# Amos-Chen98/neo-planner

Measured on NVIDIA B200. Metric: optimized trajectories/sec to convergence, higher is better.
Workload: dtype f64

## Files before the change

### neo_planner_b200/csrc/lbfgsb_tile.cuh

```cuda
#pragma once
#include "minco_tile.cuh"
#include "x87_nrm2.h"

namespace neo {

#ifdef NEO_OPT_TICKS
#define OT_BEGIN long long ot_last = clock64()
#define OT(i) do { const long long ot_now = clock64(); if (T.tl == 0) { atomicAdd((unsigned long long *)&g_opt_ticks[i], (unsigned long long)(ot_now - ot_last)); atomicAdd((unsigned long long *)&g_opt_ticks[32 + (i)], 1ull); } ot_last = clock64(); } while (0)
#else
#define OT_BEGIN do { } while (0)
#define OT(i) do { } while (0)
#endif

__device__ __forceinline__ double xmul(double a, double b) { return __dmul_rn(a, b); }
__device__ __forceinline__ double xadd(double a, double b) { return __dadd_rn(a, b); }
__device__ __forceinline__ double xsub(double a, double b) { return __dsub_rn(a, b); }
__device__ __noinline__ double xdiv(double a, double b) { return __ddiv_rn(a, b); }
__device__ __noinline__ double xsqrt(double a) { return __dsqrt_rn(a); }
__device__ __noinline__ double nrm2_x87(int n, const double *v) { return x87_nrm2(n, v); }
__device__ __forceinline__ double xrcp(double a) { return __drcp_rn(a); }
__device__ __forceinline__ double xfma(double a, double b, double c) { return __fma_rn(a, b, c); }
__device__ __forceinline__ double xdiv_r(double a, double b, double rb)
{
    const double q = __dmul_rn(a, rb);
    return __fma_rn(__fma_rn(-b, q, a), rb, q);
}

struct Dcsrch {
    bool brackt;
    int stage;
    double finit, ginit, gtest, width, width1, stx, fx, gx, sty, fy, gy, stmin, stmax;
};

#define LS_FTOL 1e-3
#define LS_GTOL 0.9
#define LS_XTOL 0.1
#define LS_STPMIN 0.0
#define LS_STPMAX 1e10

__device__ __forceinline__ double max3(double a, double b, double c) { return fmax(a, fmax(b, c)); }

__device__ __forceinline__ void dcstep(double &stx, double &fx, double &dx, double &sty, double &fy, double &dy, double &stp,
                                       double fp, double dp, bool &brackt, double stpmin, double stpmax)
{
    const double sgnd = xmul(dp, dx > 0.0 ? 1.0 : (dx < 0.0 ? -1.0 : __longlong_as_double(0x7ff8000000000000LL)));
    const int kase = fp > fx ? 1 : (sgnd < 0.0 ? 2 : (fabs(dp) < fabs(dx) ? 3 : 4));
    const bool cubic = kase < 4 || brackt;
    const double fa = kase < 4 ? fx : fp, fb = kase < 4 ? fp : fy, da = kase < 4 ? dx : dy;
    const double den = kase < 4 ? xsub(stp, stx) : xsub(sty, stp);
    double theta = 0.0, gamma = 0.0, rden = 0.0;
    if (cubic) {
        rden = __drcp_rn(den);
        theta = xadd(xadd(xdiv_r(xmul(3.0, xsub(fa, fb)), den, rden), da), dp);
        const double s = max3(fabs(theta), fabs(da), fabs(dp));
        const double rs = __drcp_rn(s);
        const double ts = xdiv_r(theta, s, rs);
        double rad = xsub(xmul(ts, ts), xmul(xdiv_r(da, s, rs), xdiv_r(dp, s, rs)));
        if (kase == 3) rad = fmax(0.0, rad);
        gamma = xmul(s, __dsqrt_rn(rad));
        const bool flip = kase == 1 ? stp < stx : (kase == 4 ? stp > sty : stp > stx);
        if (flip) gamma = -gamma;
    }
    const double g1 = xsub(gamma, kase == 1 ? dx : dp);
    const double p = xadd(g1, theta);
    const double q = kase == 3 ? xadd(xadd(gamma, xsub(dx, dp)), gamma) : xadd(xadd(g1, gamma), kase == 1 ? dp : (kase == 2 ? dx : dy));
    const double r = cubic ? __ddiv_rn(p, q) : 0.0;
    const double qn = kase == 1 ? dx : dp;
    const double qd = kase == 1 ? xadd(xdiv_r(xsub(fx, fp), den, rden), dx) : xsub(dp, dx);
    const double qq = kase < 4 ? __ddiv_rn(qn, qd) : 0.0;
    double stpf, stpc, stpq;
    if (kase == 1) {
        stpc = xadd(stx, xmul(r, den));
        stpq = xadd(stx, xmul(xmul(qq, 0.5), den));
        if (fabs(xsub(stpc, stx)) < fabs(xsub(stpq, stx))) stpf = stpc; else stpf = xadd(stpc, xmul(xsub(stpq, stpc), 0.5));
        brackt = true;
    } else if (kase == 2) {
        stpc = xadd(stp, xmul(r, xsub(stx, stp)));
        stpq = xadd(stp, xmul(qq, xsub(stx, stp)));
        if (fabs(xsub(stpc, stp)) > fabs(xsub(stpq, stp))) stpf = stpc; else stpf = stpq;
        brackt = true;
    } else if (kase == 3) {
        if (r < 0.0 && gamma != 0.0) stpc = xadd(stp, xmul(r, xsub(stx, stp)));
        else if (stp > stx) stpc = stpmax;
        else stpc = stpmin;
        stpq = xadd(stp, xmul(qq, xsub(stx, stp)));
        if (brackt) {
            if (fabs(xsub(stpc, stp)) < fabs(xsub(stpq, stp))) stpf = stpc; else stpf = stpq;
            if (stp > stx) stpf = fmin(xadd(stp, xmul(0.66, xsub(sty, stp))), stpf);
            else stpf = fmax(xadd(stp, xmul(0.66, xsub(sty, stp))), stpf);
        } else {
            if (fabs(xsub(stpc, stp)) > fabs(xsub(stpq, stp))) stpf = stpc; else stpf = stpq;
            stpf = fmin(stpmax, stpf); stpf = fmax(stpmin, stpf);
        }
    } else {
        if (brackt) stpf = xadd(stp, xmul(r, xsub(sty, stp)));
        else if (stp > stx) stpf = stpmax;
        else stpf = stpmin;
    }
    if (fp > fx) { sty = stp; fy = fp; dy = dp; }
    else {
        if (sgnd < 0.0) { sty = stx; fy = fx; dy = dx; }
        stx = stp; fx = fp; dx = dp;
    }
    stp = stpf;
}

__device__ __forceinline__ void dcsrch_start(Dcsrch &S, double stp, double f, double g)
{
    S.brackt = false; S.stage = 1; S.finit = f; S.ginit = g; S.gtest = xmul(LS_FTOL, g);
    S.width = LS_STPMAX - LS_STPMIN; S.width1 = xmul(S.width, 2.0);
    S.stx = 0.0; S.fx = f; S.gx = g; S.sty = 0.0; S.fy = f; S.gy = g;
    S.stmin = 0.0; S.stmax = xadd(stp, xmul(4.0, stp));
}

__device__ __forceinline__ int dcsrch_step(Dcsrch &S, double &stp, double f, double g)
{
    const double ftest = xadd(S.finit, xmul(stp, S.gtest));
    int task = 0;
    if (S.stage == 1 && f <= ftest && g >= 0.0) S.stage = 2;
    if (S.brackt && (stp <= S.stmin || stp >= S.stmax)) task = 2;
    if (S.brackt && xsub(S.stmax, S.stmin) <= xmul(LS_XTOL, S.stmax)) task = 2;
    if (stp == LS_STPMAX && f <= ftest && g <= S.gtest) task = 2;
    if (stp == LS_STPMIN && (f > ftest || g >= S.gtest)) task = 2;
    if (f <= ftest && fabs(g) <= xmul(LS_GTOL, -S.ginit)) task = 1;
    if (task) return task;
    {
        const bool mod = S.stage == 1 && f <= S.fx && f > ftest;
        const double gt = mod ? S.gtest : 0.0;
        const double fm = xsub(f, xmul(stp, gt)), gm = xsub(g, gt);
        double fxm = xsub(S.fx, xmul(S.stx, gt)), fym = xsub(S.fy, xmul(S.sty, gt)), gxm = xsub(S.gx, gt), gym = xsub(S.gy, gt);
        dcstep(S.stx, fxm, gxm, S.sty, fym, gym, stp, fm, gm, S.brackt, S.stmin, S.stmax);
        S.fx = xadd(fxm, xmul(S.stx, gt)); S.fy = xadd(fym, xmul(S.sty, gt));
        S.gx = xadd(gxm, gt); S.gy = xadd(gym, gt);
    }
    if (S.brackt) {
        if (fabs(xsub(S.sty, S.stx)) >= xmul(0.66, S.width1)) stp = xadd(S.stx, xmul(0.5, xsub(S.sty, S.stx)));
        S.width1 = S.width; S.width = fabs(xsub(S.sty, S.stx));
    }
    if (S.brackt) { S.stmin = fmin(S.stx, S.sty); S.stmax = fmax(S.stx, S.sty); }
    else { S.stmin = xadd(stp, xmul(1.1, xsub(stp, S.stx))); S.stmax = xadd(stp, xmul(4.0, xsub(stp, S.stx))); }
    stp = fmax(stp, LS_STPMIN); stp = fmin(stp, LS_STPMAX);
    if ((S.brackt && (stp <= S.stmin || stp >= S.stmax)) || (S.brackt && xsub(S.stmax, S.stmin) <= xmul(LS_XTOL, S.stmax)))
        stp = S.stx;
    return 0;
}

__device__ __noinline__ double blas_ddot(int n, const double *a, const double *b)
{
    double s = 0.0;
    int i = 0;
    if (n >= 16) {
        double v[4];
#pragma unroll
        for (int l = 0; l < 4; l++)
            v[l] = xadd(xadd(xadd(xmul(a[l], b[l]), xmul(a[4 + l], b[4 + l])), xmul(a[8 + l], b[8 + l])), xmul(a[12 + l], b[12 + l]));
        s = xadd(xadd(v[0], v[2]), xadd(v[1], v[3]));
        i = 16;
    }
#pragma unroll 1
    for (; i < n; i++) s = xfma(a[i], b[i], s);
    return s;
}
__device__ __noinline__ double loop_dot(int n, const double *a, const double *b)
{
    double s = 0.0;
#pragma unroll 1
    for (int i = 0; i < n; i++) s = xadd(s, xmul(a[i], b[i]));
    return s;
}

template <int N>
__device__ __forceinline__ double loop_dot_n(const double *a, const double *b, int n = N)
{
    if constexpr (N > 0 && N <= 10) {
        double s = 0.0;
#pragma unroll
        for (int i = 0; i < N; i++) s = xadd(s, xmul(a[i], b[i]));
        return s;
    } else return loop_dot(n, a, b);
}
template <int N>
__device__ __forceinline__ double blas_ddot_n(const double *a, const double *b, int n = N)
{
    if constexpr (N > 0 && N <= 10) {
        double s = 0.0;
#pragma unroll
        for (int i = 0; i < N; i++) s = xfma(a[i], b[i], s);
        return s;
    } else return blas_ddot(n, a, b);
}

__device__ __forceinline__ int wn_col(int j) { return j * (j + 1) / 2; }

__device__ __noinline__ bool lb_potf2(int tl, int TL, unsigned mask, double *wn, double *rd, int o, int n)
{
#pragma unroll 1
    for (int j = 0; j < n; j++) {
        double *cj = wn + wn_col(o + j) + o;
        double dot = 0.0;
#pragma unroll 1
        for (int k = 0; k < j; k++) dot = xfma(cj[k], cj[k], dot);
        const int m1 = j & ~3, k3 = j - m1;
        double v[2];
#pragma unroll
        for (int q = 0; q < 2; q++) {
            const int i = j + 1 + tl + q * TL;
            v[q] = 0.0;
            if (i < n) {
                const double *ci = wn + wn_col(o + i) + o;
                double t = ci[j];
                if (m1) {
                    double a0 = xmul(ci[0], cj[0]), a1 = xmul(ci[1], cj[1]), a2 = xmul(ci[2], cj[2]), a3 = xmul(ci[3], cj[3]);
                    if (m1 == 8) {
                        a0 = xadd(a0, xmul(ci[4], cj[4])); a1 = xadd(a1, xmul(ci[5], cj[5]));
                        a2 = xadd(a2, xmul(ci[6], cj[6])); a3 = xadd(a3, xmul(ci[7], cj[7]));
                    }
                    t = xsub(t, xadd(xadd(a0, a2), xadd(a1, a3)));
                }
                if (k3 == 1) t = xfma(ci[m1], -cj[m1], t);
                else if (k3 == 2) t = xadd(t, xfma(ci[m1], -cj[m1], xmul(ci[m1 + 1], -cj[m1 + 1])));
                else if (k3 == 3) t = xadd(t, xfma(ci[m1 + 2], -cj[m1 + 2], xfma(ci[m1], -cj[m1], xmul(ci[m1 + 1], -cj[m1 + 1]))));
                v[q] = t;
            }
        }
        double ajj = xsub(cj[j], dot);
        if (!(ajj > 0.0)) return false;
        ajj = __dsqrt_rn(ajj);
        const double r = __drcp_rn(ajj);
        __syncwarp(mask);
        if (tl == 0) { cj[j] = ajj; rd[o + j] = r; }
#pragma unroll
        for (int q = 0; q < 2; q++) {
            const int i = j + 1 + tl + q * TL;
            if (i < n) wn[wn_col(o + i) + o + j] = xmul(v[q], r);
        }
        __syncwarp(mask);
    }
    return true;
}

struct LbMem {
    int col, head, iupdat;
    double theta;
};

__device__ __forceinline__ int lb_slot(const LbMem &L, int k) { const int s = L.head + k; return s >= HIST ? s - HIST : s; }

template <int TL, int NC>
__device__ __forceinline__ void lb_update(const Tile<TL> &T, const TileMem &m, int n, LbMem &L, double s, double y, double rr, double dr)
{
    OT_BEGIN;
    L.iupdat++;
    if (L.iupdat <= HIST) L.col = L.iupdat;
    else L.head = L.head + 1 == HIST ? 0 : L.head + 1;
    const int col = L.col, slot = lb_slot(L, col - 1);
    if (T.tl < n) { m.ws[slot * n + T.tl] = s; m.wy[slot * n + T.tl] = y; }
    L.theta = xdiv(rr, dr);
    if (T.tl == 0) m.dr[slot] = dr;
    T.sync();
    const double *ynew = m.wy + slot * n;
#pragma unroll 1
    for (int e = T.tl; e < 2 * col; e += TL) {
        if (e < col) {
            const int sj = lb_slot(L, e);
            m.yr[slot * HIST + sj] = loop_dot_n<NC>(ynew, m.wy + sj * n, n);
        } else {
            const int si = lb_slot(L, e - col);
            const double v = loop_dot_n<NC>(m.ws + si * n, ynew, n);
            if (si == slot) m.rzd[slot] = v; else m.yr[si * HIST + slot] = v;
        }
    }
    T.sync();
    OT(2);
}

template <int TL>
__device__ __forceinline__ bool lb_factor(const Tile<TL> &T, const TileMem &m, const LbMem &L)
{
    const int col = L.col;
    OT_BEGIN;
    const double theta = L.theta, rtheta = xrcp(theta);
    double *wn = m.wn, *rd = m.wn + wn_col(LBW) + LBW;
#pragma unroll 1
    for (int iy = T.tl; iy < col; iy += TL) {
        const int si = lb_slot(L, iy), is = col + iy;
        double *c1 = wn + wn_col(iy), *c2 = wn + wn_col(is);
#pragma unroll 1
        for (int jy = 0; jy <= iy; jy++) {
            const int sj = lb_slot(L, jy);
            double v = xdiv_r(m.yr[si * HIST + sj], theta, rtheta);
            if (jy == iy) v = xadd(v, m.dr[si]);
            c1[jy] = v;
            c2[col + jy] = 0.0;
        }
#pragma unroll 1
        for (int jy = 0; jy < iy; jy++) c2[jy] = -0.0;
#pragma unroll 1
        for (int jy = iy; jy < col; jy++) {
            const int sj = lb_slot(L, jy);
            c2[jy] = jy == iy ? m.rzd[si] : m.yr[si * HIST + sj];
        }
    }
    T.sync();
    OT(3);
    if (!lb_potf2(T.tl, TL, T.mask, wn, rd, 0, col)) return false;
    OT(4);
    if (col == 1) {
        if (T.tl == 0) wn[wn_col(1)] = xdiv_r(wn[wn_col(1)], wn[0], rd[0]);
    } else {
#pragma unroll 1
        for (int c = col + T.tl; c < 2 * col; c += TL) {
            double *b = wn + wn_col(c);
            int kk = 0;
#pragma unroll 1
            for (int bs = 8; bs > 0; bs >>= 1) {
                if (!(col & bs)) continue;
                if (kk > 0)
#pragma unroll 1
                    for (int i = kk; i < kk + bs; i++) {
                        const double *ui = wn + wn_col(i);
                        double acc = 0.0;
#pragma unroll 1
                        for (int k = 0; k < kk; k++) acc = xfma(ui[k], b[k], acc);
                        b[i] = xsub(b[i], acc);
                    }
#pragma unroll 1
                for (int i = kk; i < kk + bs; i++) {
                    b[i] = xmul(b[i], rd[i]);
#pragma unroll 1
                    for (int k = i + 1; k < kk + bs; k++) b[k] = xfma(-b[i], wn[wn_col(k) + i], b[k]);
                }
                kk += bs;
            }
        }
    }
    T.sync();
    OT(5);
#pragma unroll 1
    for (int e = T.tl; e < col * (col + 1) / 2; e += TL) {
        int jj = 0;
        while ((jj + 1) * (jj + 2) / 2 <= e) jj++;
        const int ii = e - jj * (jj + 1) / 2, js = col + jj, is = col + ii;
        wn[wn_col(js) + is] = xadd(wn[wn_col(js) + is], blas_ddot(col, wn + wn_col(is), wn + wn_col(js)));
    }
    T.sync();
    OT(6);
    const bool pd = lb_potf2(T.tl, TL, T.mask, wn, rd, col, col);
    OT(7);
    return pd;
}

template <int TL, int NC>
__device__ __forceinline__ double lb_step(const Tile<TL> &T, const TileMem &m, int n, const LbMem &L, double g)
{
    const int col = L.col, m2 = 2 * col;
    OT_BEGIN;
    const double theta = L.theta, rtheta = xrcp(theta);
    double *wn = m.wn, *wv = m.wn + wn_col(LBW), *rd = wv + LBW;
    double d = -g;
    if (T.tl < n) m.dv[T.tl] = d;
    T.sync();
#pragma unroll 1
    for (int e = T.tl; e < m2; e += TL)
        wv[e] = e < col ? loop_dot_n<NC>(m.wy + lb_slot(L, e) * n, m.dv, n) : xmul(theta, loop_dot_n<NC>(m.ws + lb_slot(L, e - col) * n, m.dv, n));
    T.sync();
    OT(8);
    {
        constexpr int RPL = (LBW + TL - 1) / TL;
        double s[RPL];
#pragma unroll
        for (int q = 0; q < RPL; q++) s[q] = 0.0;
#pragma unroll 1
        for (int k = 0; k < m2; k++) {
            if ((k & (TL - 1)) == T.tl) {
                double v = wv[k];
                if (k > 0) {
                    double sk = s[0];
#pragma unroll
                    for (int q = 1; q < RPL; q++) if (k / TL == q) sk = s[q];
                    v = xsub(v, sk);
                }
                wv[k] = xdiv_r(v, wn[wn_col(k) + k], rd[k]);
            }
            T.sync();
            const double bk = wv[k];
#pragma unroll
            for (int q = 0; q < RPL; q++) {
                const int r = T.tl + q * TL;
                if (r > k && r < m2) {
                    const double *ur = wn + wn_col(r);
                    if (r < 16 || k >= 16) s[q] = xfma(ur[k], bk, s[q]);
                    else if (k == 15) s[q] = blas_ddot(16, ur, wv);
                }
            }
        }
    }
    T.sync();
    OT(9);
#pragma unroll 1
    for (int i = T.tl; i < col; i += TL) wv[i] = -wv[i];
    T.sync();
#pragma unroll 1
    for (int i = m2 - 1; i >= 0; i--) {
        const double *ui = wn + wn_col(i);
        if (T.tl == 0) wv[i] = xdiv_r(wv[i], ui[i], rd[i]);
        T.sync();
        const double t = -wv[i];
#pragma unroll 1
        for (int k = T.tl; k < i; k += TL) wv[k] = xfma(t, ui[k], wv[k]);
        T.sync();
    }
    OT(10);
    if (T.tl < n) {
#pragma unroll 1
        for (int jy = 0; jy < col; jy++) {
            const int sj = lb_slot(L, jy);
            d = xadd(xadd(d, xdiv_r(xmul(m.wy[sj * n + T.tl], wv[jy]), theta, rtheta)), xmul(m.ws[sj * n + T.tl], wv[col + jy]));
        }
        d = xmul(d, rtheta);
    }
    T.sync();
    OT(11);
    return d;
}

template <int TL>
__device__ __forceinline__ void ls_load(const Tile<TL> &T, const double *p, Dcsrch &S)
{
    S.finit = p[0]; S.ginit = p[1]; S.gtest = p[2]; S.width = p[3]; S.width1 = p[4]; S.stx = p[5]; S.fx = p[6]; S.gx = p[7];
    S.sty = p[8]; S.fy = p[9]; S.gy = p[10]; S.stmin = p[11]; S.stmax = p[12];
    const int flags = (int)p[13];
    S.brackt = (flags & 1) != 0; S.stage = flags >> 1;
}
template <int TL>
__device__ __forceinline__ void ls_store(const Tile<TL> &T, double *p, const Dcsrch &S)
{
    T.sync();
    if (T.tl == 0) {
        p[0] = S.finit; p[1] = S.ginit; p[2] = S.gtest; p[3] = S.width; p[4] = S.width1; p[5] = S.stx; p[6] = S.fx; p[7] = S.gx;
        p[8] = S.sty; p[9] = S.fy; p[10] = S.gy; p[11] = S.stmin; p[12] = S.stmax;
        p[13] = (double)((S.brackt ? 1 : 0) | (S.stage << 1));
    }
    T.sync();
}

constexpr int ST_CANCELLED = 7;
constexpr int ST_RUNNING = -1;

struct OptState {
    double x, g, d, t, r, z, xlast;
    double f, stp, gd;
    LbMem L;
    int nit, nfev, ifun, status;
    bool first;
};

__device__ __forceinline__ void opt_begin(OptState &o, double x0l)
{
    o.x = x0l; o.g = 0.0; o.d = 0.0; o.t = 0.0; o.r = 0.0; o.z = 0.0; o.xlast = 0.0;
    o.f = 0.0; o.stp = 0.0; o.gd = 0.0;
    o.L.col = 0; o.L.head = 0; o.L.iupdat = 0; o.L.theta = 1.0;
    o.nit = 0; o.nfev = 0; o.ifun = 0; o.status = ST_RUNNING; o.first = true;
}

template <int TL>
__device__ __forceinline__ bool opt_same_point(const Tile<TL> &T, const OptState &o, int n)
{
    return !o.first && T.all(T.tl >= n || o.x == o.xlast);
}

template <int TL, int NC>
__device__ __forceinline__ double opt_gd(const Tile<TL> &T, const TileMem &m, int n, double g, double d)
{
    T.sync();
    if (T.tl < n) { m.gv[T.tl] = g; m.dv[T.tl] = d; }
    T.sync();
    return blas_ddot_n<NC>(m.gv, m.dv, n);
}

template <int TL, int NC>
__device__ __forceinline__ void opt_advance(const Tile<TL> &T, const TileMem &m, int n, OptState &o,
                                            const unsigned *cancel_word, unsigned cancel_mask)
{
    const bool mine = T.tl < n;
    const double pgtol = 1e-4, ftol = 1e-4, epsmch = 2.220446049250313e-16;
    const double tol = (ftol / epsmch) * epsmch;
    const int maxls = 20, maxiter = 15000, maxfun = 15000;
    bool new_dir;
    OT_BEGIN;
    if (o.first) {
        o.first = false;
        if (T.dmax(mine ? fabs(o.g) : 0.0) <= pgtol) { o.status = 1; return; }
        new_dir = true;
    } else {
        o.gd = opt_gd<TL, NC>(T, m, n, o.g, o.d);
        Dcsrch ls;
        ls_load(T, m.ls, ls);
        const int ls_task = dcsrch_step(ls, o.stp, o.f, o.gd);
        if (ls_task == 0) ls_store(T, m.ls, ls);
        OT(0);
        if (ls_task == 0) new_dir = false;
        else {
            o.nit++;
            if (cancel_mask) {
                unsigned w = 0;
                if (T.tl == 0) w = *reinterpret_cast<const volatile unsigned *>(cancel_word);
                if (T.shfl(w, 0) & cancel_mask) { o.status = ST_CANCELLED; return; }
            }
            if (T.dmax(mine ? fabs(o.g) : 0.0) <= pgtol) { o.status = 1; return; }
            const double fold = m.ls[14], gdold = m.ls[15];
            if (xsub(fold, o.f) <= xmul(tol, max3(fabs(fold), fabs(o.f), 1.0))) { o.status = 0; return; }
            if (o.nit >= maxiter || o.nfev > maxfun) { o.status = 3; return; }
            const double y = xsub(o.g, o.r);
            T.sync();
            if (mine) m.dv[T.tl] = y;
            T.sync();
            OT(12);
            const double nr = nrm2_x87(n, m.dv);
            const double rr = xmul(nr, nr);
            OT(1);
            double dr, ddum, s;
            if (o.stp == 1.0) { dr = xsub(o.gd, gdold); ddum = -gdold; s = o.d; }
            else { dr = xmul(xsub(o.gd, gdold), o.stp); s = xmul(o.d, o.stp); ddum = xmul(-gdold, o.stp); }
            if (!(dr <= xmul(epsmch, ddum))) lb_update<TL, NC>(T, m, n, o.L, s, y, rr, dr);
            new_dir = true;
        }
    }
    for (;;) {
        if (new_dir) {
            OT(15);
            if (o.L.col > 0 && !lb_factor(T, m, o.L)) { o.L.col = 0; o.L.head = 0; o.L.iupdat = 0; o.L.theta = 1.0; }
            if (o.L.col == 0) o.z = xsub(o.x, o.g);
            else o.z = xadd(o.x, lb_step<TL, NC>(T, m, n, o.L, o.g));
            o.d = mine ? xsub(o.z, o.x) : 0.0;
            T.sync();
            if (mine) m.dv[T.tl] = o.d;
            T.sync();
            OT(13);
            const double dnorm = nrm2_x87(n, m.dv);
            OT(1);
            o.stp = (o.nit == 0) ? fmin(xdiv(1.0, dnorm), LS_STPMAX) : 1.0;
            o.t = o.x; o.r = o.g;
            o.gd = opt_gd<TL, NC>(T, m, n, o.g, o.d);
            T.sync();
            if (T.tl == 0) { m.ls[14] = o.f; m.ls[15] = o.gd; }
            o.ifun = 0;
            if (o.gd >= 0.0) o.ifun = maxls + 1;
            else { Dcsrch ls; dcsrch_start(ls, o.stp, o.f, o.gd); ls_store(T, m.ls, ls); }
            OT(14);
        }
        o.ifun++;
        if (o.ifun - 1 < maxls) break;
        T.sync();
        o.x = o.t; o.g = o.r; o.f = m.ls[14];
        if (o.L.col == 0) { o.status = 2; return; }
        o.L.col = 0; o.L.head = 0; o.L.iupdat = 0; o.L.theta = 1.0;
        new_dir = true;
    }
    o.x = (o.stp == 1.0) ? o.z : xadd(xmul(o.stp, o.d), o.t);
}

}
```

Measured before the change: 2.450 million.

## Restructure Cholesky and triangular solves to cut warp barriers and pipeline direction update

Rewrites lb_potf2 so each lane keeps running squared-sum accumulators for the rows it owns, and the diagonal owner computes sqrt and reciprocal itself. This leaves one warp barrier per column instead of two and removes the serial per-column dot loop. The forward solve in lb_step now broadcasts each solved element with a shuffle instead of a shared-memory write plus sync. The final direction accumulation software-pipelines its loads one step ahead. Host-side harness files are added to check that results still match the oracle, since the new accumulation order must stay bitwise consistent.

Measured after the change: 2.413 million (median of 6 runs). 0.985x the previous value.

```diff
diff --git a/devtools/direction_host.cpp b/devtools/direction_host.cpp
--- /dev/null
+++ b/devtools/direction_host.cpp
@@ -0,0 +1,135 @@
+#include <cmath>
+#include <condition_variable>
+#include <cstdio>
+#include <cstdlib>
+#include <cstring>
+#include <mutex>
+#include <thread>
+#include <vector>
+
+#define __device__
+#define __host__
+#define __forceinline__ inline
+#define __noinline__ __attribute__((noinline))
+#define NEO_HOST_TILE
+
+static inline double __dmul_rn(double a, double b) { return a * b; }
+static inline double __dadd_rn(double a, double b) { return a + b; }
+static inline double __dsub_rn(double a, double b) { return a - b; }
+static inline double __ddiv_rn(double a, double b) { return a / b; }
+static inline double __drcp_rn(double a) { return 1.0 / a; }
+static inline double __dsqrt_rn(double a) { return std::sqrt(a); }
+static inline double __fma_rn(double a, double b, double c) { return std::fma(a, b, c); }
+static inline double __longlong_as_double(long long v) { double d; memcpy(&d, &v, sizeof d); return d; }
+
+namespace neo {
+constexpr int HIST = 10;
+constexpr int LBW = 2 * HIST;
+constexpr int WN_DOUBLES = LBW * (LBW + 1) / 2 + 2 * LBW + 2;
+
+struct LaneSeq {
+    std::mutex m;
+    std::condition_variable cv;
+    int TL = 0, turn = 0, arrived = 0, descending = 0;
+    long gen = 0;
+    double val[32] = {}, seen[32] = {};
+    int first() const { return descending ? TL - 1 : 0; }
+    int next(int lane) const { return descending ? lane - 1 : lane + 1; }
+    double exchange(int lane, double v, int src)
+    {
+        std::unique_lock<std::mutex> lk(m);
+        val[lane] = v;
+        const long g = gen;
+        if (++arrived == TL) {
+            arrived = 0; gen++;
+            for (int l = 0; l < TL; l++) seen[l] = val[l];
+            turn = first();
+        } else turn = next(lane);
+        cv.notify_all();
+        if (!cv.wait_for(lk, std::chrono::seconds(20), [&] { return gen != g && turn == lane; })) {
+            fprintf(stderr, "direction_host: lanes disagree on the number of tile barriers\n");
+            abort();
+        }
+        return seen[src];
+    }
+    void start(int lane)
+    {
+        std::unique_lock<std::mutex> lk(m);
+        cv.wait(lk, [&] { return turn == lane; });
+    }
+    void leave(int lane)
+    {
+        exchange(lane, 0.0, 0);
+        std::unique_lock<std::mutex> lk(m);
+        turn = next(lane);
+        cv.notify_all();
+    }
+};
+thread_local LaneSeq *t_seq = nullptr;
+thread_local int t_lane = 0;
+}
+
+#define __syncwarp(mask) ((void)(mask), (void)neo::t_seq->exchange(neo::t_lane, 0.0, 0))
+
+namespace neo {
+template <int TL>
+struct Tile {
+    int tl;
+    unsigned mask;
+    explicit Tile(int lane) : tl(lane), mask(~0u) {}
+    void sync() const { __syncwarp(mask); }
+    double shfl(double v, int src) const { return t_seq->exchange(tl, v, src); }
+};
+struct TileMem {
+    double *ws, *wy, *yr, *rzd, *dr, *gv, *dv, *ls, *wn;
+};
+}
+
+
+#include "../neo_planner_b200/csrc/lbfgsb_tile.cuh"
+
+template <int TL>
+static int run_tile(int descending, int n, int pairs, const double *s, const double *y, const double *rr, const double *dr,
+                    const double *g, double *wn_out, double *d)
+{
+    using namespace neo;
+    std::vector<double> ws(HIST * n), wy(HIST * n), yr(HIST * HIST), rzd(HIST), drv(HIST), gv(n), dv(n), ls(16), wn(WN_DOUBLES);
+    const TileMem m{ws.data(), wy.data(), yr.data(), rzd.data(), drv.data(), gv.data(), dv.data(), ls.data(), wn.data()};
+    LaneSeq seq;
+    seq.TL = TL; seq.descending = descending; seq.turn = seq.first();
+    int ok = 0;
+    std::vector<std::thread> lanes;
+    for (int lane = 0; lane < TL; lane++)
+        lanes.emplace_back([&, lane] {
+            t_seq = &seq; t_lane = lane;
+            seq.start(lane);
+            const Tile<TL> T(lane);
+            LbMem L{0, 0, 0, 1.0};
+            for (int k = 0; k < pairs; k++)
+                lb_update<TL, 0>(T, m, n, L, lane < n ? s[k * n + lane] : 0.0, lane < n ? y[k * n + lane] : 0.0, rr[k], dr[k]);
+            const bool pd = lb_factor(T, m, L);
+            if (pd) {
+                const double dl = lb_step<TL, 0>(T, m, n, L, lane < n ? g[lane] : 0.0);
+                if (lane < n) d[lane] = dl;
+            }
+            if (lane == 0) ok = pd;
+            if (lane == 0 && pd) {
+                for (int j = 0; j < 2 * L.col; j++)
+                    for (int i = 0; i <= j; i++) wn_out[i * LBW + j] = wn[wn_col(j) + i];
+            }
+            seq.leave(lane);
+        });
+    for (auto &t : lanes) t.join();
+    return ok;
+}
+
+extern "C" int device_direction(int TL, int descending, int n, int pairs, const double *s, const double *y,
+                                const double *rr, const double *dr, const double *g, double *wn, double *d)
+{
+    switch (TL) {
+        case 8: return run_tile<8>(descending, n, pairs, s, y, rr, dr, g, wn, d);
+        case 16: return run_tile<16>(descending, n, pairs, s, y, rr, dr, g, wn, d);
+        case 32: return run_tile<32>(descending, n, pairs, s, y, rr, dr, g, wn, d);
+    }
+    return -1;
+}
diff --git a/devtools/direction_oracle.c b/devtools/direction_oracle.c
--- /dev/null
+++ b/devtools/direction_oracle.c
@@ -0,0 +1,13 @@
+#include "../oracle/minco_oracle.c"
+
+int oracle_direction(int n, int pairs, const double *s, const double *y, const double *rr, const double *dr,
+                     const double *g, double *wn, double *d)
+{
+    static __thread lb_mem C;
+    lb_reset(&C, n);
+    for (int k = 0; k < pairs; k++) lb_update(&C, s + (size_t)k * n, y + (size_t)k * n, rr[k], dr[k]);
+    const int ok = lb_factor(&C);
+    memcpy(wn, C.wn, sizeof(C.wn));
+    if (ok) lb_step(&C, g, d);
+    return ok;
+}
diff --git a/neo_planner_b200/csrc/lbfgsb_tile.cuh b/neo_planner_b200/csrc/lbfgsb_tile.cuh
--- a/neo_planner_b200/csrc/lbfgsb_tile.cuh
+++ b/neo_planner_b200/csrc/lbfgsb_tile.cuh
@@ -1,5 +1,7 @@
 #pragma once
+#ifndef NEO_HOST_TILE
 #include "minco_tile.cuh"
+#endif
 #include "x87_nrm2.h"
 
 namespace neo {
@@ -194,20 +196,25 @@
 
 __device__ __noinline__ bool lb_potf2(int tl, int TL, unsigned mask, double *wn, double *rd, int o, int n)
 {
+    double dot0 = 0.0, dot1 = 0.0;
 #pragma unroll 1
     for (int j = 0; j < n; j++) {
-        double *cj = wn + wn_col(o + j) + o;
-        double dot = 0.0;
-#pragma unroll 1
-        for (int k = 0; k < j; k++) dot = xfma(cj[k], cj[k], dot);
+        if ((j & (TL - 1)) == tl) {
+            double *ujj = wn + wn_col(o + j) + o + j;
+            const double u = __dsqrt_rn(xsub(*ujj, j < TL ? dot0 : dot1));
+            *ujj = u;
+            rd[o + j] = __drcp_rn(u);
+        }
+        __syncwarp(mask);
+        const double *cj = wn + wn_col(o + j) + o;
+        if (!(cj[j] > 0.0)) return false;
+        const double r = rd[o + j];
         const int m1 = j & ~3, k3 = j - m1;
-        double v[2];
-#pragma unroll
+#pragma unroll 1
         for (int q = 0; q < 2; q++) {
-            const int i = j + 1 + tl + q * TL;
-            v[q] = 0.0;
-            if (i < n) {
-                const double *ci = wn + wn_col(o + i) + o;
+            const int i = tl + q * TL;
+            if (i > j && i < n) {
+                double *ci = wn + wn_col(o + i) + o;
                 double t = ci[j];
                 if (m1) {
                     double a0 = xmul(ci[0], cj[0]), a1 = xmul(ci[1], cj[1]), a2 = xmul(ci[2], cj[2]), a3 = xmul(ci[3], cj[3]);
@@ -220,21 +227,12 @@
                 if (k3 == 1) t = xfma(ci[m1], -cj[m1], t);
                 else if (k3 == 2) t = xadd(t, xfma(ci[m1], -cj[m1], xmul(ci[m1 + 1], -cj[m1 + 1])));
                 else if (k3 == 3) t = xadd(t, xfma(ci[m1 + 2], -cj[m1 + 2], xfma(ci[m1], -cj[m1], xmul(ci[m1 + 1], -cj[m1 + 1]))));
-                v[q] = t;
+                const double u = xmul(t, r);
+                ci[j] = u;
+                dot0 = xfma(u, u, dot0);
             }
-        }
-        double ajj = xsub(cj[j], dot);
-        if (!(ajj > 0.0)) return false;
-        ajj = __dsqrt_rn(ajj);
-        const double r = __drcp_rn(ajj);
-        __syncwarp(mask);
-        if (tl == 0) { cj[j] = ajj; rd[o + j] = r; }
-#pragma unroll
-        for (int q = 0; q < 2; q++) {
-            const int i = j + 1 + tl + q * TL;
-            if (i < n) wn[wn_col(o + i) + o + j] = xmul(v[q], r);
-        }
-        __syncwarp(mask);
+            const double t = dot0; dot0 = dot1; dot1 = t;
+        }
     }
     return true;
 }
@@ -277,6 +275,7 @@
 template <int TL>
 __device__ __forceinline__ bool lb_factor(const Tile<TL> &T, const TileMem &m, const LbMem &L)
 {
+    static_assert(2 * TL >= HIST, "lb_potf2 keeps at most two columns per lane");
     const int col = L.col;
     OT_BEGIN;
     const double theta = L.theta, rtheta = xrcp(theta);
@@ -372,6 +371,7 @@
         for (int q = 0; q < RPL; q++) s[q] = 0.0;
 #pragma unroll 1
         for (int k = 0; k < m2; k++) {
+            double bk = 0.0;
             if ((k & (TL - 1)) == T.tl) {
                 double v = wv[k];
                 if (k > 0) {
@@ -380,10 +380,11 @@
                     for (int q = 1; q < RPL; q++) if (k / TL == q) sk = s[q];
                     v = xsub(v, sk);
                 }
-                wv[k] = xdiv_r(v, wn[wn_col(k) + k], rd[k]);
+                bk = xdiv_r(v, wn[wn_col(k) + k], rd[k]);
+                wv[k] = bk;
             }
-            T.sync();
-            const double bk = wv[k];
+            bk = T.shfl(bk, k & (TL - 1));
+            if (k == 15 && m2 > 16) T.sync();
 #pragma unroll
             for (int q = 0; q < RPL; q++) {
                 const int r = T.tl + q * TL;
@@ -395,8 +396,8 @@
             }
         }
     }
-    T.sync();
     OT(9);
+    T.sync();
 #pragma unroll 1
     for (int i = T.tl; i < col; i += TL) wv[i] = -wv[i];
     T.sync();
@@ -412,10 +413,19 @@
     }
     OT(10);
     if (T.tl < n) {
+        const double *wyl = m.wy + T.tl, *wsl = m.ws + T.tl;
+        int sj = lb_slot(L, 0) * n;
+        double p = xdiv_r(xmul(wyl[sj], wv[0]), theta, rtheta), q = xmul(wsl[sj], wv[col]);
 #pragma unroll 1
         for (int jy = 0; jy < col; jy++) {
-            const int sj = lb_slot(L, jy);
-            d = xadd(xadd(d, xdiv_r(xmul(m.wy[sj * n + T.tl], wv[jy]), theta, rtheta)), xmul(m.ws[sj * n + T.tl], wv[col + jy]));
+            double pn = 0.0, qn = 0.0;
+            if (jy + 1 < col) {
+                sj = lb_slot(L, jy + 1) * n;
+                pn = xdiv_r(xmul(wyl[sj], wv[jy + 1]), theta, rtheta);
+                qn = xmul(wsl[sj], wv[col + jy + 1]);
+            }
+            d = xadd(xadd(d, p), q);
+            p = pn; q = qn;
         }
         d = xmul(d, rtheta);
     }
```
